# Greketrotny/RayZath

Measured on AMD Instinct MI355X. Metric: Mrays/s (path segments, primary+secondary) at 1920x1080 depth 8, higher is better.
Workload: dtype f32; 1 GPU; Cornell box 1920x1080 depth 8; max_depth=8, triangles=16, instances=8, traversal=workgroup-binned, integrator=CPU kernel (parity-checked), pipeline=resident (one kernel per step)

## Files before the change

### rayzath_amd/csrc/hiprz_device.hpp

```cpp
#pragma once
#include <hip/hip_runtime.h>
#include <stdint.h>

#include "hiprz.h"
#include "hiprz_end.hpp"
#include "hiprz_lds.hpp"
#include "hiprz_shard.hpp"

#define RZ_DEV __device__ __forceinline__
#include "hiprz_flat_pick.hpp"
#include "hiprz_pair_pick.hpp"
#include "hiprz_u8_div.hpp"

namespace hiprz {

#ifndef RZ_FUSED_SHARED_RCP
#define RZ_FUSED_SHARED_RCP 0
#endif
#ifndef RZ_TRACE_SHARED_RCP
#define RZ_TRACE_SHARED_RCP 1
#endif
#ifndef RZ_BATCH_SHARED_RCP
#define RZ_BATCH_SHARED_RCP 1
#endif
#ifndef RZ_MIRROR_LOBE_CONST
#define RZ_MIRROR_LOBE_CONST 1
#endif
#ifndef RZ_TRACE_MIN_WAVES
#define RZ_TRACE_MIN_WAVES 5
#endif
#define RZ_PI_F 3.14159265358979323846f
#define RZ_GUARD_LIMIT (1u << 26)
#ifndef RZ_WALK_GUARD
#define RZ_WALK_GUARD 0
#endif
#if RZ_WALK_GUARD
#define RZ_GUARD(counter) \
    if (++(counter) > RZ_GUARD_LIMIT) break
#else
#define RZ_GUARD(counter) (void)(counter)
#endif
#define RZ_FLT_MAX 3.402823466e+38f

#define RZ_SINF(x) sinf(x)
#define RZ_COSF(x) cosf(x)
#define RZ_SINCOSF(x, s, c) sincosf((x), &(s), &(c))
#define RZ_ACOSF(x) acosf(x)
#define RZ_ASINF(x) asinf(x)
#define RZ_ATAN2F(y, x) atan2f(y, x)
#define RZ_POWF(x, y) powf(x, y)
#define RZ_EXPF(x) expf(x)
#define RZ_LOGF(x) logf(x)

struct DScene {
    const float4* nodes;
    const uint32_t* tlas_order;
    const float4* tris;
    const float4* tri_attrs;
    const float4* instances;
    const int32_t* inst_materials;
    const float4* materials;
    const float4* textures;
    const uint8_t* texels;
    const float4* spot_lights;
    const float4* direct_lights;
    uint32_t n_instances;
    uint32_t tlas_root;
    uint32_t n_spot_lights;
    uint32_t n_direct_lights;
    uint32_t fast_div;
    uint32_t hot_bytes;
    const float4* hot;
    uint32_t off_nodes, off_tlas_order, off_instances, off_tris, off_tri_attrs, off_materials, off_inst_materials;
    uint32_t world_stack_entries;
    uint32_t mesh_stack_entries;
    float bounds_min[3];
    float bounds_scale[3];
    uint32_t top_count;
    const uint32_t* node_skip;
    uint32_t walk_k, walk_l;
    uint32_t walk_advance;
    uint32_t world_advance;
    uint32_t walk_h;
    uint32_t off_pairs;
    const float4* nodes64;
    uint32_t shadow_variant;
    const float4* shadow_nodes64;
    const uint32_t* shadow_order;
    uint32_t shadow_root;
    uint32_t sort_variant;
};

RZ_DEV void repoint_hot(DScene& v, const unsigned char* base) {
    v.nodes = reinterpret_cast<const float4*>(base + v.off_nodes);
    v.tlas_order = reinterpret_cast<const uint32_t*>(base + v.off_tlas_order);
    v.instances = reinterpret_cast<const float4*>(base + v.off_instances);
    v.tris = reinterpret_cast<const float4*>(base + v.off_tris);
    v.tri_attrs = reinterpret_cast<const float4*>(base + v.off_tri_attrs);
    v.materials = reinterpret_cast<const float4*>(base + v.off_materials);
    v.inst_materials = reinterpret_cast<const int32_t*>(base + v.off_inst_materials);
}

static_assert(sizeof(DScene) == 256, "off_pairs fills a padding word: the kernels' argument layout is what it was");
RZ_DEV const unsigned char* pair_section(const DScene& s) { return reinterpret_cast<const unsigned char*>(s.nodes) - s.off_nodes + s.off_pairs; }

#ifndef RZ_SURFACE_RECORDS
#define RZ_SURFACE_RECORDS 1
#endif
RZ_DEV const float4* surface_section(const DScene& s) { return s.hot + ((s.hot_bytes + 15u) >> 4); }

struct DCamera {
    float position[3];
    float x_axis[3], y_axis[3], z_axis[3];
    uint32_t width, height;
    float tan_half_fov, aspect_ratio;
    float near_, far_;
    float focal_distance, aperture, exposure_time;
};

struct DConfig {
    uint32_t max_depth, spot_samples, direct_samples, seed;
    uint32_t flags;
};

struct DFrame {
    float4* st0;
    float4* st1;
    float2* st2;
    float4* accum;
    float4* hit0;
    uint32_t* hit1;
    float* depth;
    uint32_t* rgba8;
    const uint32_t* pass;
    unsigned long long* counters;
    uint32_t tiles_x;
    uint32_t rank, world;
    uint32_t n_local_tiles;
    uint32_t* sort_key;
    const uint32_t* perm;
    uint32_t xcd_swizzle;
    float4* nee;
    uint32_t nee_quads;
    uint32_t* shadow_key;
    const uint32_t* shadow_perm;
    const uint32_t* launch_order;
    uint32_t* unit_cost;
};
constexpr uint32_t kSegFlags = 4u;
constexpr uint32_t kSegWaitLimit = 1u << 22;

struct v3 {
    float x, y, z;
};
struct col4 {
    float r, g, b, a;
};

RZ_DEV v3 V3(float x, float y, float z) { return v3{x, y, z}; }
RZ_DEV v3 ld3(const float* p) { return v3{p[0], p[1], p[2]}; }
RZ_DEV v3 xyz(float4 f) { return v3{f.x, f.y, f.z}; }
RZ_DEV v3 operator+(v3 a, v3 b) { return v3{a.x + b.x, a.y + b.y, a.z + b.z}; }
RZ_DEV v3 operator-(v3 a, v3 b) { return v3{a.x - b.x, a.y - b.y, a.z - b.z}; }
// ... 455 lines not shown
    return hit.instance >= 0 ? 2 : 1;
}

template <bool COUNT>
RZ_DEV float any_hit_stack(const DScene& s, uint32_t* lds_column, const Ray& ray, Counters& cnt) {
    LdsStack w(lds_column);
    const bool scene_fast = s.fast_div != 0u;
    WalkRay g;
    g.o = ray.o, g.d = ray.d, g.near_ = ray.near_, g.far_ = ray.far_;
    prepare<false>(g, scene_fast);
    uint32_t n = s.tlas_root, guard = 0u;
    while (n != RZ_END) {
        RZ_GUARD(guard);
        const float4 n0 = s.nodes[2 * n], n1 = s.nodes[2 * n + 1];
        RZ_COUNT(box_tests);
        RZ_COUNT(shadow_box_tests);
        if (box_hit<false>(n0, n1, g)) {
            const uint32_t begin = __float_as_uint(n1.z), meta = __float_as_uint(n1.w);
            if (!(meta & HIPRZ_NODE_LEAF)) {
                n = w.descend(begin);
                continue;
            }
            const uint32_t end = begin + (meta & HIPRZ_NODE_COUNT_MASK);
            for (uint32_t i = begin; i < end; ++i) {
                const uint32_t inst = s.tlas_order[i];
                float4 ib0, ib1;
                load_instance_box(s, inst, ib0, ib1);
                RZ_COUNT(box_tests);
        RZ_COUNT(shadow_box_tests);
                if (!box_hit<false>(ib0, ib1, g)) continue;
                const InstanceXform x = load_instance_xform(s, inst);
                WalkRay lr;
                to_local<false>(x, g, lr, scene_fast);
                const uint32_t base = w.mark();
                uint32_t m = x.blas_root;
                while (m != RZ_END) {
                    RZ_GUARD(guard);
                    const float4 m0 = s.nodes[2 * m], m1 = s.nodes[2 * m + 1];
                    RZ_COUNT(box_tests);
        RZ_COUNT(shadow_box_tests);
                    if (box_hit<false>(m0, m1, lr)) {
                        const uint32_t mbegin = __float_as_uint(m1.z), mmeta = __float_as_uint(m1.w);
                        if (!(mmeta & HIPRZ_NODE_LEAF)) {
                            m = w.descend(mbegin);
                            continue;
                        }
                        const uint32_t mend = mbegin + (mmeta & HIPRZ_NODE_COUNT_MASK);
                        for (uint32_t j = mbegin; j < mend; ++j) {
                            const float4 a = s.tris[3 * j], b = s.tris[3 * j + 1], c = s.tris[3 * j + 2];
                            float t, b1, b2, det;
                            RZ_COUNT(tri_tests);
                            RZ_COUNT(shadow_tri_tests);
                            if (tri_hit(xyz(a), xyz(b), xyz(c), lr, t, b1, b2, det)) return 0.0f;
                        }
                    }
                    m = w.next(base);
                }
            }
        } else if (n == s.tlas_root) {
            return 1.0f;
        }
        n = w.next(0u);
    }
    return 1.0f;
}


#define RZ_BIN_NONE 0xFFFFFFFFu
#define RZ_BIN_WIDE 0x80000000u
RZ_DEV uint32_t octet_min(uint32_t v);
struct BinnedLds {
    float* ray;
    uint32_t* hit;
    uint32_t* items;
    uint32_t* bins;
    uint32_t* stacks;
    static constexpr uint32_t kFixedBytes = kBinnedFixedBytes;
    static __host__ uint32_t bytes_host(uint32_t world_entries, uint32_t mesh_entries) {
        return kFixedBytes + (world_entries + mesh_entries) * kBinnedEntryBytes;
    }
    __device__ __forceinline__ explicit BinnedLds(unsigned char* base) {
        ray = reinterpret_cast<float*>(base);
        hit = reinterpret_cast<uint32_t*>(base + 8u * 1024u);
        items = reinterpret_cast<uint32_t*>(base + 13u * 1024u);
        bins = reinterpret_cast<uint32_t*>(base + 14u * 1024u);
        stacks = reinterpret_cast<uint32_t*>(base + kFixedBytes);
    }
};

struct FlatWorld {
    float4 root0, root1;
    uint32_t ids;
    uint32_t count;
    uint32_t wide;
};
RZ_DEV uint32_t wave_uniform(uint32_t v) { return uint32_t(__builtin_amdgcn_readfirstlane(int(v))); }
RZ_DEV float wave_uniform(float v) { return __uint_as_float(wave_uniform(__float_as_uint(v))); }
RZ_DEV float4 wave_uniform(float4 v) { return make_float4(wave_uniform(v.x), wave_uniform(v.y), wave_uniform(v.z), wave_uniform(v.w)); }
RZ_DEV FlatWorld make_flat_world(const DScene& s) {
    FlatWorld fw;
    fw.root0 = fw.root1 = make_float4(0.0f, 0.0f, 0.0f, 0.0f);
    fw.ids = fw.count = fw.wide = 0u;
    if (s.n_instances == 0) return fw;
    fw.root0 = wave_uniform(s.nodes[2 * s.tlas_root]), fw.root1 = wave_uniform(s.nodes[2 * s.tlas_root + 1]);
    const uint32_t begin = __float_as_uint(fw.root1.z);
    fw.count = __float_as_uint(fw.root1.w) & HIPRZ_NODE_COUNT_MASK;
    if (fw.count > 8u) fw.count = 8u;
#pragma unroll
    for (uint32_t k = 0; k < 8u; ++k)
        if (k < fw.count) fw.ids = flat_pack_id(fw.ids, k, wave_uniform(s.tlas_order[begin + k]));
    const uint32_t i = threadIdx.x & 63u;
    bool wide = false;
    if (i < s.n_instances && i < 8u) {
        const uint32_t root = __float_as_uint(s.instances[7 * i].w);
        const uint32_t meta = __float_as_uint(s.nodes[2 * root + 1].w);
        wide = (meta & HIPRZ_NODE_LEAF) != 0u && (meta & HIPRZ_NODE_COUNT_MASK) > 4u;
    }
    fw.wide = uint32_t(__ballot(wide)) & 0xFFu;
    return fw;
}

template <bool COUNT, bool RCP>
RZ_DEV uint32_t pretest_leaf_instances(const DScene& s, const FlatWorld& fw, const WalkRay& g, float (&tm)[8], bool counting, Counters& cnt) {
    uint32_t mask = 0u;
    if (fw.count == 8u && RCP && __all(g.fast)) {
#pragma unroll
        for (uint32_t k = 0; k < 8u; ++k) {
            float4 ib0, ib1;
            load_instance_box(s, flat_id(fw.ids, k), ib0, ib1);
            float tmin, tmax;
            box_range_fast(ib0, ib1, g, tmin, tmax);
            if (counting) { RZ_PHASE(1); RZ_COUNT(box_tests); }
            mask |= uint32_t(!(tmax < g.near_ || tmin > tmax)) << k;
            tm[k] = tmin;
        }
        return mask;
    }
#pragma unroll
    for (uint32_t k = 0; k < 8u; ++k) {
        tm[k] = 0.0f;
        if (k < fw.count) {
            float4 ib0, ib1;
            load_instance_box(s, flat_id(fw.ids, k), ib0, ib1);
            float tmin, tmax;
            box_range_unpacked<RCP>(ib0, ib1, g, tmin, tmax);
            if (counting) { RZ_PHASE(1); RZ_COUNT(box_tests); }
            mask |= uint32_t(!(tmax < g.near_ || tmin > tmax)) << k;
            tm[k] = tmin;
        }
    }
    return mask;
}

template <bool COUNT, bool RCP>
RZ_DEV void binned_visit(const DScene& s, const BinnedLds& lds, uint32_t* mesh_column, bool scene_fast, uint32_t slot, Counters& cnt) {
    RZ_PHASE(2);
    const uint32_t item = lds.items[slot], inst = (item & 0x7FFFFFFFu) >> 8, src = item & 255u;
    WalkRay w;
    w.o = V3(lds.ray[0 * 256 + src], lds.ray[1 * 256 + src], lds.ray[2 * 256 + src]);
    w.d = V3(lds.ray[3 * 256 + src], lds.ray[4 * 256 + src], lds.ray[5 * 256 + src]);
    w.near_ = lds.ray[6 * 256 + src], w.far_ = lds.ray[7 * 256 + src];
    const InstanceXform x = load_instance_xform(s, inst);
    WalkRay lr;
    const float len = to_local<RCP>(x, w, lr, scene_fast);
    const float4 n0 = s.nodes[2 * x.blas_root], n1 = s.nodes[2 * x.blas_root + 1];
    const bool wide = (item & RZ_BIN_WIDE) != 0u;
    if (wide || (__float_as_uint(n1.w) & HIPRZ_NODE_LEAF) != 0u) {
        const uint32_t j = wide ? slot & 7u : 0u;
        RZ_PHASE(3);
        if (j == 0u) { RZ_COUNT(box_tests); }
        LeafBest best;
        best.far_ = lr.far_, best.triangle = 0xFFFFFFFFu, best.b1 = best.b2 = 0.0f, best.external = false;
        if (box_hit_unpacked<RCP>(n0, n1, lr)) {
            const uint32_t begin = __float_as_uint(n1.z), end = begin + (__float_as_uint(n1.w) & HIPRZ_NODE_COUNT_MASK);
            const uint32_t count = end - begin, n_pairs = (count + 1u) >> 1;
            const unsigned char* section = pair_section(s);
            const float2* rec = reinterpret_cast<const float2*>(section + 8u * reinterpret_cast<const uint16_t*>(section)[inst]);
            for (uint32_t p = j; p < n_pairs; p += wide ? 8u : 1u) {
                const float2* q = rec + p * (RZ_PAIR_RECORD_BYTES / 8u);
                const float2 v1x = q[0], v1y = q[1], v1z = q[2], e1x = q[3], e1y = q[4], e1z = q[5], e2x = q[6], e2y = q[7], e2z = q[8];
                const bool has_b = 2u * p + 1u < count;
                const uint32_t i = begin + 2u * p;
                RZ_PHASE(4);
                if constexpr (COUNT) cnt.tri_tests += has_b ? 2u : 1u;
                tri_pair_step(v3p{f2{v1x.x, v1x.y}, f2{v1y.x, v1y.y}, f2{v1z.x, v1z.y}}, v3p{f2{e1x.x, e1x.y}, f2{e1y.x, e1y.y}, f2{e1z.x, e1z.y}},
                              v3p{f2{e2x.x, e2x.y}, f2{e2y.x, e2y.y}, f2{e2z.x, e2z.y}}, i, has_b, lr, best);
            }
        }
        bool mine = best.triangle != 0xFFFFFFFFu;
        if (wide) {
            const uint32_t wide_t = mine ? __float_as_uint(best.far_) : 0xFFFFFFFFu;
            const uint32_t t_min = octet_min(wide_t);
            const bool nearest = wide_t != 0xFFFFFFFFu && wide_t == t_min;
            const uint32_t first = octet_min(nearest ? best.triangle : 0xFFFFFFFFu);
            mine = nearest && best.triangle == first;
        }
        if (mine) {
            lds.ray[6 * 256 + src] = lr.near_ / len;
            lds.ray[7 * 256 + src] = best.far_ / len;
            lds.hit[0 * 256 + src] = best.triangle;
            lds.hit[1 * 256 + src] = best.external ? 1u : 0u;
            lds.hit[2 * 256 + src] = __float_as_uint(best.b1);
            lds.hit[3 * 256 + src] = __float_as_uint(best.b2);
            lds.hit[4 * 256 + src] = inst;
        }
        return;
    }
    LdsStack mesh(mesh_column);
    Hit h;
    if (closest_in_mesh_stack<COUNT, RCP, false>(s, mesh, x.blas_root, lr, h, cnt)) {
        lds.ray[6 * 256 + src] = lr.near_ / len;
        lds.ray[7 * 256 + src] = lr.far_ / len;
        lds.hit[0 * 256 + src] = h.triangle;
        lds.hit[1 * 256 + src] = h.external ? 1u : 0u;
        lds.hit[2 * 256 + src] = __float_as_uint(h.bx);
        lds.hit[3 * 256 + src] = __float_as_uint(h.by);
        lds.hit[4 * 256 + src] = inst;
    }
}

template <bool COUNT, bool RCP>
__device__ __forceinline__ int closest_hit_binned(const DScene& s, unsigned char* workspace, bool active, Ray& ray, Hit& hit,
                                                  Counters& cnt) {
    const uint32_t tid = threadIdx.x;
    BinnedLds lds(workspace);
    hit.instance = -1, hit.triangle = 0, hit.bx = hit.by = 0.0f, hit.external = true;
    if (s.n_instances == 0) return 0;

    lds.ray[0 * 256 + tid] = ray.o.x, lds.ray[1 * 256 + tid] = ray.o.y, lds.ray[2 * 256 + tid] = ray.o.z;
    lds.ray[3 * 256 + tid] = ray.d.x, lds.ray[4 * 256 + tid] = ray.d.y, lds.ray[5 * 256 + tid] = ray.d.z;
    lds.ray[6 * 256 + tid] = ray.near_, lds.ray[7 * 256 + tid] = ray.far_;
    lds.hit[4 * 256 + tid] = 0xFFFFFFFFu;

    LdsStack world(lds.stacks + tid);
    uint32_t* mesh_column = lds.stacks + s.world_stack_entries * 256u + tid;
    const bool sorted = s.n_instances <= 64u;
    WalkRay g;
    g.o = ray.o, g.d = ray.d, g.near_ = ray.near_, g.far_ = ray.far_;
    const bool scene_fast = s.fast_div != 0u;
    prepare<RCP>(g, scene_fast);
    uint32_t n = active ? s.tlas_root : RZ_END;
    uint32_t leaf_i = 0, leaf_end = 0;
    bool root_missed = false;
    uint32_t round = 0u;
    if (tid < 128u) lds.bins[tid] = 0u;
    unsigned long long wide_mask = 0ull;
    if (sorted) {
        const uint32_t k = tid & 63u;
        bool wide = false;
        if (k < s.n_instances) {
            const uint32_t root = __float_as_uint(s.instances[7 * k].w);
            const uint32_t meta = __float_as_uint(s.nodes[2 * root + 1].w);
            wide = (meta & HIPRZ_NODE_LEAF) != 0u && (meta & HIPRZ_NODE_COUNT_MASK) > 4u;
        }
        wide_mask = __ballot(wide);
    }
    __syncthreads();

    uint32_t guard = 0u;
    while (round < (1u << 20)) {
        RZ_PHASE(5);
        uint32_t cand = RZ_BIN_NONE;
        while (true) {
            RZ_GUARD(guard);
            if (leaf_i < leaf_end) {
                const uint32_t inst = s.tlas_order[leaf_i++];
                float4 ib0, ib1;
                load_instance_box(s, inst, ib0, ib1);
                RZ_PHASE(1);
                RZ_COUNT(box_tests);
                if (box_hit_unpacked<RCP>(ib0, ib1, g)) {
                    cand = inst;
                    break;
                }
                continue;
            }
            if (n == RZ_END) break;
            const float4 n0 = s.nodes[2 * n], n1 = s.nodes[2 * n + 1];
            RZ_PHASE(0);
            RZ_COUNT(box_tests);
            if (box_hit_unpacked<RCP>(n0, n1, g)) {
                const uint32_t begin = __float_as_uint(n1.z), meta = __float_as_uint(n1.w);
                if (!(meta & HIPRZ_NODE_LEAF)) {
                    n = world.descend(begin);
                    continue;
                }
                leaf_i = begin, leaf_end = begin + (meta & HIPRZ_NODE_COUNT_MASK);
            } else if (n == s.tlas_root) {
                root_missed = true;
            }
            n = world.next(0u);
        }

        uint32_t* bins = lds.bins + (round & 1u) * 64u;
        uint32_t rank = 0u;
        const uint32_t bin = sorted ? cand : 0u;
        const bool wide_item = cand != RZ_BIN_NONE && cand < 64u && ((wide_mask >> cand) & 1ull) != 0ull;
        if (cand != RZ_BIN_NONE) rank = atomicAdd(&bins[bin], wide_item ? 8u : 1u);
        __syncthreads();
        const uint32_t lane = tid & 63u;
        const uint32_t c = bins[lane];
        const bool wide_bin = ((wide_mask >> lane) & 1ull) != 0ull;
        uint32_t incl = wide_bin ? (c | ((c >> 3) << 21)) : ((c << 12) | (c << 21));
        const uint32_t own = incl;
#pragma unroll
        for (int off = 1; off < 64; off <<= 1) {
            const uint32_t v = __shfl_up(incl, off);
            if (int(lane) >= off) incl += v;
        }
        const uint32_t totals = __shfl(incl, 63);
        const uint32_t n_visits = totals >> 21;
        if (n_visits == 0u) break;
        const uint32_t wide_lanes = totals & 0xFFFu, narrow_lanes = (totals >> 12) & 0x1FFu;
        const bool split = wide_lanes != 0u && wide_lanes + narrow_lanes <= 256u;
        const uint32_t n_items = split ? wide_lanes + narrow_lanes : n_visits;
        const uint32_t before = __shfl(incl - own, int(bin & 63u));
        if (cand != RZ_BIN_NONE) {
            if (split && wide_item) {
                const uint32_t at = (before & 0xFFFu) + rank;
#pragma unroll
                for (uint32_t j = 0; j < 8u; ++j) lds.items[at + j] = RZ_BIN_WIDE | (cand << 8) | tid;
            } else if (split) {
                lds.items[wide_lanes + ((before >> 12) & 0x1FFu) + rank] = (cand << 8) | tid;
            } else {
                lds.items[(before >> 21) + (wide_item ? rank >> 3 : rank)] = (cand << 8) | tid;
            }
        }
        if (tid < 64u) lds.bins[((round + 1u) & 1u) * 64u + tid] = 0u;
        __syncthreads();

        const uint32_t slot = (tid - ((blockIdx.x + round) & 3u) * 64u) & 255u;
        if (slot < n_items) {
            RZ_PHASE(2);
            const uint32_t item = lds.items[slot], inst = (item & 0x7FFFFFFFu) >> 8, src = item & 255u;
            WalkRay w;
            w.o = V3(lds.ray[0 * 256 + src], lds.ray[1 * 256 + src], lds.ray[2 * 256 + src]);
// ... 3 lines not shown
            WalkRay lr;
            const float len = to_local<RCP>(x, w, lr, scene_fast);
            if (item & RZ_BIN_WIDE) {
                const uint32_t j = slot & 7u;
                const float4 n0 = s.nodes[2 * x.blas_root], n1 = s.nodes[2 * x.blas_root + 1];
                RZ_PHASE(3);
                if (j == 0u) { RZ_COUNT(box_tests); }
                uint32_t wide_t = 0xFFFFFFFFu, wide_tri = 0xFFFFFFFFu;
                float wide_b1 = 0.0f, wide_b2 = 0.0f;
                bool wide_external = false;
                const float visit_near = lr.near_;
                if (box_hit_unpacked<RCP>(n0, n1, lr)) {
                    const uint32_t begin = __float_as_uint(n1.z), end = begin + (__float_as_uint(n1.w) & HIPRZ_NODE_COUNT_MASK);
                    for (uint32_t i = begin + j; i < end; i += 8u) {
                        const float4 a = s.tris[3 * i], b = s.tris[3 * i + 1], cc = s.tris[3 * i + 2];
                        float t, b1, b2, det;
                        RZ_PHASE(4);
                        RZ_COUNT(tri_tests);
                        if (tri_hit(xyz(a), xyz(b), xyz(cc), lr, t, b1, b2, det)) {
                            lr.far_ = t;
                            wide_t = __float_as_uint(t), wide_tri = i, wide_b1 = b1, wide_b2 = b2, wide_external = det > 0.0f;
                        }
                    }
                }
                const uint32_t t_min = octet_min(wide_t);
                const bool nearest = wide_t != 0xFFFFFFFFu && wide_t == t_min;
                const uint32_t first = octet_min(nearest ? wide_tri : 0xFFFFFFFFu);
                if (nearest && wide_tri == first) {
                    lds.ray[6 * 256 + src] = visit_near / len;
                    lds.ray[7 * 256 + src] = __uint_as_float(wide_t) / len;
                    lds.hit[0 * 256 + src] = wide_tri;
                    lds.hit[1 * 256 + src] = wide_external ? 1u : 0u;
                    lds.hit[2 * 256 + src] = __float_as_uint(wide_b1);
                    lds.hit[3 * 256 + src] = __float_as_uint(wide_b2);
                    lds.hit[4 * 256 + src] = inst;
                }
            } else {
                LdsStack mesh(mesh_column);
                Hit h;
                if (closest_in_mesh_stack<COUNT, RCP, false>(s, mesh, x.blas_root, lr, h, cnt)) {
                    lds.ray[6 * 256 + src] = lr.near_ / len;
                    lds.ray[7 * 256 + src] = lr.far_ / len;
                    lds.hit[0 * 256 + src] = h.triangle;
                    lds.hit[1 * 256 + src] = h.external ? 1u : 0u;
                    lds.hit[2 * 256 + src] = __float_as_uint(h.bx);
                    lds.hit[3 * 256 + src] = __float_as_uint(h.by);
                    lds.hit[4 * 256 + src] = inst;
                }
            }
        }
        __syncthreads();
        round += 1u;
        g.near_ = lds.ray[6 * 256 + tid];
        g.far_ = lds.ray[7 * 256 + tid];
    }
    ray.o = V3(lds.ray[0 * 256 + tid], lds.ray[1 * 256 + tid], lds.ray[2 * 256 + tid]);
    ray.d = V3(lds.ray[3 * 256 + tid], lds.ray[4 * 256 + tid], lds.ray[5 * 256 + tid]);
    ray.near_ = g.near_, ray.far_ = g.far_;
    const uint32_t inst = lds.hit[4 * 256 + tid];
    if (inst != 0xFFFFFFFFu) {
        hit.instance = int32_t(inst);
        hit.triangle = lds.hit[0 * 256 + tid];
        hit.external = lds.hit[1 * 256 + tid] != 0u;
        hit.bx = __uint_as_float(lds.hit[2 * 256 + tid]);
        hit.by = __uint_as_float(lds.hit[3 * 256 + tid]);
    }
    if (root_missed) return 0;
    return hit.instance >= 0 ? 2 : 1;
}


struct DppShr {
    template <int N>
    __device__ __forceinline__ uint32_t operator()(uint32_t v, FlatShift<N>) const {
        return uint32_t(__builtin_amdgcn_update_dpp(0, int(v), 0x110 + N, 0xF, 0xF, true));
    }
};
template <bool COUNT, bool RCP>
__device__ __forceinline__ int closest_hit_flat(const DScene& s, const FlatWorld& fw, unsigned char* workspace, bool active, Ray& ray, Hit& hit,
                                                Counters& cnt) {
    const uint32_t tid = threadIdx.x;
    BinnedLds lds(workspace);
    hit.instance = -1, hit.triangle = 0, hit.bx = hit.by = 0.0f, hit.external = true;
    if (s.n_instances == 0) return 0;

    lds.ray[0 * 256 + tid] = ray.o.x, lds.ray[1 * 256 + tid] = ray.o.y, lds.ray[2 * 256 + tid] = ray.o.z;
    lds.ray[3 * 256 + tid] = ray.d.x, lds.ray[4 * 256 + tid] = ray.d.y, lds.ray[5 * 256 + tid] = ray.d.z;
    lds.ray[6 * 256 + tid] = ray.near_, lds.ray[7 * 256 + tid] = ray.far_;
    lds.hit[4 * 256 + tid] = 0xFFFFFFFFu;

    uint32_t* mesh_column = lds.stacks + s.world_stack_entries * 256u + tid;
    WalkRay g;
    g.o = ray.o, g.d = ray.d, g.near_ = ray.near_, g.far_ = ray.far_;
    const bool scene_fast = s.fast_div != 0u;
    prepare<RCP>(g, scene_fast);
    bool root_missed = false;
    uint32_t round = 0u;
    float tm[8] = {0.0f, 0.0f, 0.0f, 0.0f, 0.0f, 0.0f, 0.0f, 0.0f};
    uint32_t flat_mask = 0u, flat_next = 0u;
    float flat_near = g.near_;
    if (active) {
        RZ_PHASE(0);
        RZ_COUNT(box_tests);
        if (box_hit_unpacked<RCP>(fw.root0, fw.root1, g)) flat_mask = pretest_leaf_instances<COUNT, RCP>(s, fw, g, tm, true, cnt);
        else root_missed = true;
    }
    if (tid < 128u) lds.bins[tid] = 0u;
    __syncthreads();

    const uint32_t lane = tid & 63u;
    const bool wide_bin = ((fw.wide >> (lane & 7u)) & 1u) != 0u;
    while (round < (1u << 20)) {
        RZ_PHASE(5);
        if (__any(flat_mask != 0u && __float_as_uint(g.near_) != __float_as_uint(flat_near))) {
            if (flat_mask != 0u && __float_as_uint(g.near_) != __float_as_uint(flat_near)) {
                WalkRay t;
                t.o = V3(lds.ray[0 * 256 + tid], lds.ray[1 * 256 + tid], lds.ray[2 * 256 + tid]);
                t.d = V3(lds.ray[3 * 256 + tid], lds.ray[4 * 256 + tid], lds.ray[5 * 256 + tid]);
                t.near_ = g.near_, t.far_ = g.far_;
                prepare<RCP>(t, scene_fast);
                flat_mask = pretest_leaf_instances<COUNT, RCP>(s, fw, t, tm, false, cnt) & flat_from(flat_next);
                flat_near = g.near_;
            }
        }
        const uint32_t cand = flat_pick(fw.ids, tm, g.far_, flat_mask, flat_next);

        uint32_t* bins = lds.bins + (round & 1u) * 64u;
        uint32_t rank = 0u;
        const bool wide_item = cand != kFlatNone && ((fw.wide >> cand) & 1u) != 0u;
        if (cand != kFlatNone) rank = atomicAdd(&bins[cand], wide_item ? 8u : 1u);
        __syncthreads();
        const uint32_t c = bins[lane];
        if (!__any(c != 0u)) break;
        const uint32_t own = flat_pack_bin(c, wide_bin);
        const uint32_t incl = flat_prefix8(own, DppShr{});
        const FlatRound r = flat_round(uint32_t(__builtin_amdgcn_readlane(int(incl), 7)));
#ifdef RZ_PHASE_STATS
        if (!r.split) { RZ_PHASE(6); }
#endif
        const uint32_t before = __shfl(incl - own, int(cand & 7u));
        if (cand != kFlatNone) {
            const uint32_t at = flat_item_slot(r, before, rank, wide_item);
            if (r.split && wide_item) {
#pragma unroll
                for (uint32_t j = 0; j < 8u; ++j) lds.items[at + j] = RZ_BIN_WIDE | (cand << 8) | tid;
            } else {
                lds.items[at] = (cand << 8) | tid;
            }
        }
        if (tid < 64u) lds.bins[((round + 1u) & 1u) * 64u + tid] = 0u;
        __syncthreads();

        const uint32_t slot = (tid - ((blockIdx.x + round) & 3u) * 64u) & 255u;
        if (slot < r.n_items) {
            binned_visit<COUNT, RCP>(s, lds, mesh_column, scene_fast, slot, cnt);
        }
        __syncthreads();
        round += 1u;
        g.near_ = lds.ray[6 * 256 + tid];
        g.far_ = lds.ray[7 * 256 + tid];
    }
    ray.o = V3(lds.ray[0 * 256 + tid], lds.ray[1 * 256 + tid], lds.ray[2 * 256 + tid]);
    ray.d = V3(lds.ray[3 * 256 + tid], lds.ray[4 * 256 + tid], lds.ray[5 * 256 + tid]);
    ray.near_ = g.near_, ray.far_ = g.far_;
    const uint32_t inst = lds.hit[4 * 256 + tid];
    if (inst != 0xFFFFFFFFu) {
        hit.instance = int32_t(inst);
        hit.triangle = lds.hit[0 * 256 + tid];
        hit.external = lds.hit[1 * 256 + tid] != 0u;
        hit.bx = __uint_as_float(lds.hit[2 * 256 + tid]);
        hit.by = __uint_as_float(lds.hit[3 * 256 + tid]);
    }
    if (root_missed) return 0;
    return hit.instance >= 0 ? 2 : 1;
}


struct TopCache {
    const float4* nodes;
    const uint32_t* skip;
    uint32_t count;
    static __host__ uint32_t bytes_host(uint32_t top_count) { return top_count * kTopNodeBytes; }
};
RZ_DEV uint32_t octant_of(v3 d) { return uint32_t(d.z < 0.0f) | (uint32_t(d.y < 0.0f) << 1) | (uint32_t(d.x < 0.0f) << 2); }
RZ_DEV void fetch_node_ordered(const DScene& s, uint32_t n, uint32_t oct, float4& n0, float4& n1, uint32_t& link) {
    const float4* rec = s.nodes64 + 4 * size_t(n);
    n0 = rec[0], n1 = rec[1];
    link = reinterpret_cast<const uint32_t*>(rec + 2)[oct];
}
RZ_DEV bool tri_hit_ordered(v3 v1, v3 edge1, v3 edge2, const WalkRay& r, bool tie_ok, float& t_out, float& b1_out, float& b2_out, float& det_out) {
    const v3 pvec = cross(r.d, edge2);
    float det = dot(edge1, pvec);
    det += float(uint32_t(det > -1.0e-7f) & uint32_t(det < 1.0e-7f)) * 1.0e-7f;
    const float inv_det = 1.0f / det;
    const v3 tvec = r.o - v1;
    const float b1 = dot(tvec, pvec) * inv_det;
    if (b1 < 0.0f || b1 > 1.0f) return false;
    const v3 qvec = cross(tvec, edge1);
    const float b2 = dot(r.d, qvec) * inv_det;
    if (b2 < 0.0f || b1 + b2 > 1.0f) return false;
    const float t = dot(edge2, qvec) * inv_det;
    if (t <= r.near_ || t > r.far_ || (t == r.far_ && !tie_ok)) return false;
    t_out = t, b1_out = b1, b2_out = b2, det_out = det;
    return true;
}
RZ_DEV void fetch_node(const DScene& s, const TopCache& top, uint32_t n, float4& n0, float4& n1, uint32_t& link) {
    if (n < top.count) {
        n0 = top.nodes[2 * n], n1 = top.nodes[2 * n + 1], link = top.skip[n];
    } else {
        n0 = s.nodes[2 * n], n1 = s.nodes[2 * n + 1], link = s.node_skip[n];
    }
}
template <bool COUNT, bool RCP, bool TIES = false>
RZ_DEV int closest_hit_skip(const DScene& s, const TopCache& top, Ray& ray, Hit& hit, Counters& cnt) {
    const bool scene_fast = s.fast_div != 0u;
    WalkRay g;
    g.o = ray.o, g.d = ray.d, g.near_ = ray.near_, g.far_ = ray.far_;
    prepare<RCP>(g, scene_fast);
    uint32_t n = s.tlas_root, guard = 0u;
    while (n != RZ_END) {
        RZ_GUARD(guard);
        float4 n0, n1;
        uint32_t link;
        fetch_node(s, top, n, n0, n1, link);
        RZ_PHASE(0);
        RZ_COUNT(box_tests);
        if (box_hit<RCP>(n0, n1, g)) {
            const uint32_t begin = __float_as_uint(n1.z), meta = __float_as_uint(n1.w);
            if (!(meta & HIPRZ_NODE_LEAF)) {
                n = begin;
                continue;
            }
            uint32_t end = begin + (meta & HIPRZ_NODE_COUNT_MASK);
            for (uint32_t i = begin; i < end; ++i) {
                uint32_t inst = s.tlas_order[i];
                float4 ib0, ib1;
                load_instance_box(s, inst, ib0, ib1);
                RZ_PHASE(1);
                RZ_COUNT(box_tests);
                if (!box_hit<RCP>(ib0, ib1, g)) continue;
                RZ_PHASE(2);
                const InstanceXform x = load_instance_xform(s, inst);
                WalkRay lr;
                float len = to_local<RCP>(x, g, lr, scene_fast);
                bool found = false;
                uint32_t held_refpos = 0u;
                uint32_t m = x.blas_root;
                uint32_t tj = 0u, tj_end = 0u;
                const uint32_t kmax = s.walk_k ? s.walk_k : 0xFFFFFFFFu, lmax = s.walk_l ? s.walk_l : 0xFFFFFFFFu;
                while (true) {
                    RZ_PHASE(5);
                    uint32_t k = 0u;
                    while (tj == tj_end && m != RZ_END && k < kmax) {
                        RZ_GUARD(guard);
                        k += 1u;
                        float4 m0, m1;
                        uint32_t mlink;
                        fetch_node(s, top, m, m0, m1, mlink);
                        RZ_PHASE(3);
                        RZ_COUNT(box_tests);
                        if (box_hit<RCP>(m0, m1, lr)) {
                            const uint32_t mbegin = __float_as_uint(m1.z), mmeta = __float_as_uint(m1.w);
                            if (!(mmeta & HIPRZ_NODE_LEAF)) {
                                m = mbegin;
                                continue;
                            }
                            tj = mbegin, tj_end = mbegin + (mmeta & HIPRZ_NODE_COUNT_MASK);
                        }
                        m = mlink;
                    }
                    if (tj == tj_end && m == RZ_END) break;
                    uint32_t l = 0u;
                    for (; tj < tj_end && l < lmax; ++tj, ++l) {
                        const float4 a = s.tris[3 * tj], b = s.tris[3 * tj + 1], c = s.tris[3 * tj + 2];
                        float t, b1, b2, det;
                        RZ_PHASE(4);
                        RZ_COUNT(tri_tests);
                        const uint32_t refpos = __float_as_uint(c.w);
                        if (TIES ? tri_hit_ordered(xyz(a), xyz(b), xyz(c), lr, found && refpos < held_refpos, t, b1, b2, det)
                                 : tri_hit(xyz(a), xyz(b), xyz(c), lr, t, b1, b2, det)) {
                            lr.far_ = t;
                            hit.triangle = tj;
                            hit.external = det > 0.0f;
                            hit.bx = b1, hit.by = b2;
                            found = true, held_refpos = refpos;
                        }
                    }
                }
                if (found) {
                    hit.instance = int32_t(inst);
                    g.near_ = lr.near_ / len;
                    g.far_ = lr.far_ / len;
                }
            }
        } else if (n == s.tlas_root) {
            return 0;
        }
        n = link;
    }
    ray.near_ = g.near_, ray.far_ = g.far_;
    return hit.instance >= 0 ? 2 : 1;
}

#define RZ_LDS __attribute__((address_space(3)))
typedef float f4 __attribute__((ext_vector_type(4)));
RZ_DEV f4 F4(float x, float y, float z, float w) { return f4{x, y, z, w}; }
struct CoopLds {
// ... 1223 lines not shown
```

Measured before the change: 13430 Mrays/s.

## Redistribute long leaf triangle-pair work across idle wave lanes

Adds a dealt leaf-visit path. When few lanes in a wave own long leaves, their remaining triangle-pair tests are spread across all 64 lanes using a wave prefix sum and ds_bpermute lane pulls, and the nearest hit is then reduced back to the owning lane. It targets lane divergence, where a few rays loop over many pairs while most of the wave sits idle. The cost is extra cross-lane shuffles, a serial reduction loop over each owner's remainder, register pressure, and a more complex control path. Tie-breaking could also differ from the original order.

```diff
diff --git a/rayzath_amd/csrc/hiprz_deal_pick.hpp b/rayzath_amd/csrc/hiprz_deal_pick.hpp
--- /dev/null
+++ b/rayzath_amd/csrc/hiprz_deal_pick.hpp
@@ -0,0 +1,44 @@
+#pragma once
+#include <stdint.h>
+
+#ifndef RZ_DEV
+#define RZ_DEV inline
+#endif
+
+namespace hiprz {
+
+constexpr uint32_t kDealLanes = 64u;
+constexpr uint32_t kDealNoHit = 0xFFFFFFFFu;
+constexpr uint32_t kDealExternal = 0x80000000u;
+
+RZ_DEV uint32_t deal_chunk(uint32_t work) { return work / kDealLanes; }
+RZ_DEV uint32_t deal_lane(uint32_t work) { return work % kDealLanes; }
+RZ_DEV uint32_t deal_chunks(uint32_t total) { return (total + kDealLanes - 1u) / kDealLanes; }
+
+constexpr uint32_t kDealMaxChunks = 1u;
+constexpr uint32_t kDealMinRem = 2u * kDealMaxChunks + 1u;
+constexpr uint32_t kDealMaxOwners = kDealMaxChunks * kDealLanes / kDealMinRem;
+RZ_DEV bool deal_taken(uint32_t total, uint32_t max_rem) {
+    const uint32_t chunks = deal_chunks(total);
+    return total != 0u && chunks <= kDealMaxChunks && 2u * chunks + 1u <= max_rem;
+}
+
+template <class At>
+RZ_DEV uint32_t deal_owner(uint32_t work, const At& at) {
+    uint32_t o = 0u;
+    if (at(o + 31u) <= work) o += 32u;
+    if (at(o + 15u) <= work) o += 16u;
+    if (at(o + 7u) <= work) o += 8u;
+    if (at(o + 3u) <= work) o += 4u;
+    if (at(o + 1u) <= work) o += 2u;
+    if (at(o) <= work) o += 1u;
+    return o;
+}
+RZ_DEV uint32_t deal_pair(uint32_t work, uint32_t owner_exclusive) { return work - owner_exclusive + 1u; }
+
+RZ_DEV bool deal_nearer(uint32_t t_bits, uint32_t best_bits) { return t_bits < best_bits; }
+RZ_DEV bool deal_better(uint32_t t_bits, uint32_t triangle, uint32_t best_bits, uint32_t best_triangle) {
+    return t_bits < best_bits || (t_bits == best_bits && t_bits != kDealNoHit && (triangle & ~kDealExternal) < (best_triangle & ~kDealExternal));
+}
+
+}
diff --git a/rayzath_amd/csrc/hiprz_device.hpp b/rayzath_amd/csrc/hiprz_device.hpp
--- a/rayzath_amd/csrc/hiprz_device.hpp
+++ b/rayzath_amd/csrc/hiprz_device.hpp
@@ -9,6 +9,7 @@
 
 #define RZ_DEV __device__ __forceinline__
 #include "hiprz_flat_pick.hpp"
+#include "hiprz_deal_pick.hpp"
 #include "hiprz_pair_pick.hpp"
 #include "hiprz_u8_div.hpp"
 
@@ -770,6 +771,135 @@
     return mask;
 }
 
+RZ_DEV uint32_t lane_pull(uint32_t from_lane, uint32_t v) { return uint32_t(__builtin_amdgcn_ds_bpermute(int(from_lane << 2), int(v))); }
+RZ_DEV float lane_pull(uint32_t from_lane, float v) { return __uint_as_float(lane_pull(from_lane, __float_as_uint(v))); }
+template <int N>
+RZ_DEV uint32_t row_below(uint32_t v) {
+    return uint32_t(__builtin_amdgcn_update_dpp(0, int(v), 0x110 + N, 0xF, 0xF, true));
+}
+RZ_DEV uint32_t wave_inclusive_sum(uint32_t v, uint32_t lane) {
+    v += row_below<1>(v), v += row_below<2>(v), v += row_below<4>(v), v += row_below<8>(v);
+    const uint32_t r0 = uint32_t(__builtin_amdgcn_readlane(int(v), 15)), r1 = uint32_t(__builtin_amdgcn_readlane(int(v), 31));
+    const uint32_t r2 = uint32_t(__builtin_amdgcn_readlane(int(v), 47));
+    return v + (lane >= 16u ? r0 : 0u) + (lane >= 32u ? r1 : 0u) + (lane >= 48u ? r2 : 0u);
+}
+RZ_DEV void dealt_hit(const BinnedLds& lds, uint32_t item, float near_, float len, const LeafBest& best) {
+    const uint32_t inst = item >> 8, src = item & 255u;
+    lds.ray[6 * 256 + src] = near_ / len;
+    lds.ray[7 * 256 + src] = best.far_ / len;
+    lds.hit[0 * 256 + src] = best.triangle;
+    lds.hit[1 * 256 + src] = best.external ? 1u : 0u;
+    lds.hit[2 * 256 + src] = __float_as_uint(best.b1);
+    lds.hit[3 * 256 + src] = __float_as_uint(best.b2);
+    lds.hit[4 * 256 + src] = inst;
+}
+template <bool COUNT, bool RCP>
+RZ_DEV bool dealt_visit(const DScene& s, const BinnedLds& lds, bool scene_fast, uint32_t slot, bool has_item, Counters& cnt) {
+    const uint32_t lane = threadIdx.x & 63u;
+    const unsigned char* section = pair_section(s);
+    uint32_t item = 0u, rec_off = 0u, begin = 0u, count = 0u, n_pairs = 0u, p = 0u;
+    WalkRay lr;
+    lr.o = lr.d = lr.y = V3(0.0f, 0.0f, 0.0f), lr.near_ = lr.far_ = 0.0f, lr.fast = false;
+    float len = 1.0f;
+    bool inner = false;
+    if (has_item) {
+        item = lds.items[slot];
+        const uint32_t inst = item >> 8, src = item & 255u;
+        WalkRay w;
+        w.o = V3(lds.ray[0 * 256 + src], lds.ray[1 * 256 + src], lds.ray[2 * 256 + src]);
+        w.d = V3(lds.ray[3 * 256 + src], lds.ray[4 * 256 + src], lds.ray[5 * 256 + src]);
+        w.near_ = lds.ray[6 * 256 + src], w.far_ = lds.ray[7 * 256 + src];
+        const InstanceXform x = load_instance_xform(s, inst);
+        const float4 n0 = s.nodes[2 * x.blas_root], n1 = s.nodes[2 * x.blas_root + 1];
+        inner = (__float_as_uint(n1.w) & HIPRZ_NODE_LEAF) == 0u;
+        if (!inner) {
+            RZ_PHASE(2);
+            len = to_local<RCP>(x, w, lr, scene_fast);
+            RZ_PHASE(3);
+            RZ_COUNT(box_tests);
+            if (box_hit_unpacked<RCP>(n0, n1, lr)) {
+                begin = __float_as_uint(n1.z), count = __float_as_uint(n1.w) & HIPRZ_NODE_COUNT_MASK, n_pairs = (count + 1u) >> 1;
+                rec_off = 8u * reinterpret_cast<const uint16_t*>(section)[inst];
+            }
+        }
+    }
+    LeafBest best;
+    best.far_ = lr.far_, best.triangle = 0xFFFFFFFFu, best.b1 = best.b2 = 0.0f, best.external = false;
+    bool work = p < n_pairs;
+    bool first = true, dealt = false;
+    float own_near = 0.0f;
+    uint32_t rem = 0u, excl = 0u;
+#pragma clang loop unroll(disable)
+    while (__any(work)) {
+        if (work) {
+            const float2* q = reinterpret_cast<const float2*>(section + rec_off) + p * (RZ_PAIR_RECORD_BYTES / 8u);
+            const float2 v1x = q[0], v1y = q[1], v1z = q[2], e1x = q[3], e1y = q[4], e1z = q[5], e2x = q[6], e2y = q[7], e2z = q[8];
+            const bool has_b = 2u * p + 1u < count;
+            const uint32_t i = begin + 2u * p;
+            RZ_PHASE(4);
+#ifdef RZ_PHASE_STATS
+            if (p >= 1u) { RZ_PHASE(9); }
+            if (dealt) { RZ_PHASE(14); }
+#endif
+            if constexpr (COUNT) cnt.tri_tests += has_b ? 2u : 1u;
+            tri_pair_step(v3p{f2{v1x.x, v1x.y}, f2{v1y.x, v1y.y}, f2{v1z.x, v1z.y}}, v3p{f2{e1x.x, e1x.y}, f2{e1y.x, e1y.y}, f2{e1z.x, e1z.y}},
+                          v3p{f2{e2x.x, e2x.y}, f2{e2y.x, e2y.y}, f2{e2z.x, e2z.y}}, i, has_b, lr, best);
+        }
+        if (dealt) break;
+        p += 1u, work = p < n_pairs;
+        if (first) {
+            first = false;
+            rem = work ? n_pairs - p : 0u;
+#ifdef RZ_PHASE_STATS
+            if (rem != 0u) {
+                const uint32_t k = uint32_t(__popcll(__ballot(1)));
+                RZ_PHASE(10);
+                if (k <= 12u) { RZ_PHASE(11); } else if (k <= 25u) { RZ_PHASE(12); } else { RZ_PHASE(13); }
+            }
+#endif
+            if (__any(rem >= kDealMinRem)) {
+                const uint32_t incl = wave_inclusive_sum(rem, lane);
+                const uint32_t total = uint32_t(__builtin_amdgcn_readlane(int(incl), 63));
+                if (deal_taken(total, kDealMinRem)) {
+                    dealt = true;
+                    excl = incl - rem;
+                    if (best.triangle != 0xFFFFFFFFu) dealt_hit(lds, item, lr.near_, len, best);
+                    own_near = lr.near_;
+                    const uint32_t owner = deal_owner(lane, [&](uint32_t k) { return lane_pull(k, incl); });
+                    p = deal_pair(lane, lane_pull(owner, excl));
+                    lr.o = V3(lane_pull(owner, lr.o.x), lane_pull(owner, lr.o.y), lane_pull(owner, lr.o.z));
+                    lr.d = V3(lane_pull(owner, lr.d.x), lane_pull(owner, lr.d.y), lane_pull(owner, lr.d.z));
+                    lr.near_ = lane_pull(owner, lr.near_);
+                    best.far_ = lane_pull(owner, best.far_);
+                    best.triangle = 0xFFFFFFFFu, best.b1 = best.b2 = 0.0f, best.external = false;
+                    rec_off = lane_pull(owner, rec_off), begin = lane_pull(owner, begin), count = lane_pull(owner, count);
+                    work = lane < total;
+                }
+            }
+        }
+    }
+    if (dealt) {
+        const uint32_t res_t = best.triangle != 0xFFFFFFFFu ? __float_as_uint(best.far_) : kDealNoHit;
+        const uint32_t res_triangle = best.triangle | (best.external ? kDealExternal : 0u);
+        const float res_b1 = best.b1, res_b2 = best.b2;
+        uint32_t nearest = kDealNoHit, from = kDealNoHit;
+        for (uint32_t q = 0u; __any(q < rem); ++q) {
+            const uint32_t t = lane_pull(excl + q, res_t);
+            if (q < rem && deal_nearer(t, nearest)) nearest = t, from = excl + q;
+        }
+        const bool won = from != kDealNoHit;
+        const uint32_t at = won ? from : lane;
+        const uint32_t won_triangle = lane_pull(at, res_triangle);
+        const float won_b1 = lane_pull(at, res_b1), won_b2 = lane_pull(at, res_b2);
+        best.far_ = __uint_as_float(nearest);
+        best.triangle = won ? won_triangle & ~kDealExternal : 0xFFFFFFFFu;
+        best.external = (won_triangle & kDealExternal) != 0u;
+        best.b1 = won_b1, best.b2 = won_b2;
+        lr.near_ = own_near;
+    }
+    if (best.triangle != 0xFFFFFFFFu) dealt_hit(lds, item, lr.near_, len, best);
+    return inner;
+}
 template <bool COUNT, bool RCP>
 RZ_DEV void binned_visit(const DScene& s, const BinnedLds& lds, uint32_t* mesh_column, bool scene_fast, uint32_t slot, Counters& cnt) {
     RZ_PHASE(2);
@@ -800,6 +930,14 @@
                 const bool has_b = 2u * p + 1u < count;
                 const uint32_t i = begin + 2u * p;
                 RZ_PHASE(4);
+#ifdef RZ_PHASE_STATS
+                if (!wide && p >= 1u) { RZ_PHASE(9); }
+                if (!wide && p == 1u) {
+                    const uint32_t k = uint32_t(__popcll(__ballot(1)));
+                    RZ_PHASE(10);
+                    if (k <= 12u) { RZ_PHASE(11); } else if (k <= 25u) { RZ_PHASE(12); } else { RZ_PHASE(13); }
+                }
+#endif
                 if constexpr (COUNT) cnt.tri_tests += has_b ? 2u : 1u;
                 tri_pair_step(v3p{f2{v1x.x, v1x.y}, f2{v1y.x, v1y.y}, f2{v1z.x, v1z.y}}, v3p{f2{e1x.x, e1x.y}, f2{e1y.x, e1y.y}, f2{e1z.x, e1z.y}},
                               v3p{f2{e2x.x, e2x.y}, f2{e2y.x, e2y.y}, f2{e2z.x, e2z.y}}, i, has_b, lr, best);
@@ -1109,7 +1247,16 @@
         __syncthreads();
 
         const uint32_t slot = (tid - ((blockIdx.x + round) & 3u) * 64u) & 255u;
-        if (slot < r.n_items) {
+        const bool has_item = slot < r.n_items;
+        bool deal_wave = false;
+        if (!r.split && wave_uniform(slot & ~63u) < r.n_items) {
+            const bool long_leaf = has_item && ((fw.wide >> (lds.items[has_item ? slot : 0u] >> 8)) & 1u) != 0u;
+            const uint32_t owners = uint32_t(__popcll(__ballot(long_leaf)));
+            deal_wave = owners != 0u && owners <= kDealMaxOwners;
+        }
+        bool todo = has_item;
+        if (deal_wave) todo = dealt_visit<COUNT, RCP>(s, lds, scene_fast, slot, has_item, cnt);
+        if (todo) {
             binned_visit<COUNT, RCP>(s, lds, mesh_column, scene_fast, slot, cnt);
         }
         __syncthreads();
```

Measured after the change: 13790 Mrays/s (median of 6 runs). +2.6%, better.
